# MattAgostini/ECE1782-Smith-Waterman-CUDA

Hardware: AMD Instinct MI355X
Metric: GCUPS (DP cell updates/s) query-vs-SwissProt, 1/2/4/8 MI355X; bit-exact scores (higher is better)
Workload: dtype fp16

## Files before the change

ece1782-smith-waterman-cuda_amd/csrc/sw_capi.cpp:

```cpp
#include <hip/hip_runtime.h>

#include <algorithm>
#include <cmath>
#include <atomic>
#include <cstdio>
#include <cstdlib>
#include <cstring>
#include <numeric>
#include <string>
#include <thread>
#include <unordered_map>
#include <vector>

#include "sw_amd.h"
#include "sw_kernels.h"
#include "sw_plan.h"

namespace {

thread_local std::string g_err;

constexpr int kF16Span = 2048;

uint32_t f16_pair(int v) {
// ... 1126 lines not shown
        HIPCHECK(hipHostGetDevicePointer(reinterpret_cast<void**>(&a.trace), db->h_trace, 0));
    }
    if (p.rescue) {
        a.rescue_count = c.listA;
        a.rescue_list = c.listA + 1;
        if (p.f16) a.rescue_max = c.maxA;
        const int zero = -kF16Span + 2 * ge;
        a.sat_limit = kF16Span - zero - 2 * std::max(c.sc.max_s, 1) - 26 * ge;
        for (int j = 0; j < 32; ++j) a.f16_step[j] = f16_pair(j * ge + zero);
        a.f16_gog = f16_pair(go - ge);
        a.f16_zero = f16_pair(zero);
        a.f16_diff[0] = f16_pair(4 * ge);
        a.f16_diff[1] = f16_pair(8 * ge);
        a.f16_diff[2] = f16_pair(16 * ge);
    }
    if (p.lpt) {
        a.blk_first = p.npair;
        a.blk_quad = p.nquad;
        a.blk_tri = p.ntri ? 1 : 0;
        a.blk_tail = static_cast<int32_t>(db->nblocks) - p.ntail;
    } else if (p.npair) {
        a.blk_base = p.nr;
        a.blk_first = std::max(p.npair, p.nr);
    } else {
        a.blk_first = p.ncoop;
    }
    return SW_OK;
}

void intra_args(Scan& c) {
// ... 40 lines not shown
    return c.db->nblocks ? inter_args(c) : SW_OK;
}

struct RescueStages {
    swk::InterArgs a16, a32;
    swk::IntraArgs i16, i32;
};
RescueStages rescue_stages(const Scan& c, const swk::IntraArgs& x, const BndRows& r, bool in_launch) {
    const swplan::ScanPlan& p = c.plan;
    auto items = [](int32_t* list) { return list ? list + 1 : nullptr; };
    int32_t* const l32 = p.f16 ? c.listB : c.listA;
    RescueStages s{c.a, c.a, x, c.ia};
    s.a16.bnd_h = s.a32.bnd_h = r.h;
    s.a16.bnd_f = s.a32.bnd_f = r.f;
    s.a16.qpad = p.qpad_list;
    s.a16.rescue_list = items(c.listB);
    s.a16.rescue_count = c.listB;
    s.a16.rescue_max = nullptr;
    s.a32.prof = c.P.dev + c.P.off8;
    s.a32.qpad = p.qpad_rescue;
    s.a32.rescue_list = nullptr;
    s.a32.rescue_count = nullptr;
    s.i16.bnd_h = s.i32.bnd_h = r.lh;
    s.i16.bnd_f = s.i32.bnd_f = r.lf;
    s.i16.rescue_list = items(c.list2);
    s.i16.rescue_count = c.list2;
    if (in_launch) {
        s.a16.trace = s.a32.trace = nullptr;
        s.a32.rescue_max = nullptr;
    } else {
// ... 1113 lines not shown
```

ece1782-smith-waterman-cuda_amd/csrc/sw_int32.h:

```cpp
#pragma once

#include "sw_kernels.h"

namespace swk {

__host__ __device__ constexpr int inter_stride(int R) {
    return ((R + 16 + 15) / 16) % 2 == 1 ? ((R + 16 + 15) / 16) * 16
                                         : ((R + 16 + 15) / 16 + 1) * 16;
}

__device__ __forceinline__ int sx8(uint32_t w, int b) {
    return static_cast<int>(static_cast<int8_t>(w >> (8 * b)));
}

__device__ __forceinline__ int usub(int m, uint32_t g) {
    return static_cast<int>(__builtin_elementwise_sub_sat(static_cast<uint32_t>(m), g));
}

template <int N>
__device__ __forceinline__ uint32_t pword(const int4 (&v)[N], int w) {
    const int4 q = v[w >> 2];
    switch (w & 3) {
        case 0: return static_cast<uint32_t>(q.x);
        case 1: return static_cast<uint32_t>(q.y);
// ... 237 lines not shown
template <int RI, bool AFFINE, bool WG = true>
__device__ __forceinline__ void intra_subject(const IntraArgs& a, int sid, uint8_t* lds) {
    auto sync = [] {
        if constexpr (WG) {
            __syncthreads();
        } else {
            __builtin_amdgcn_fence(__ATOMIC_RELEASE, "workgroup");
            __builtin_amdgcn_wave_barrier();
            __builtin_amdgcn_fence(__ATOMIC_ACQUIRE, "workgroup");
        }
    };
    constexpr int CH = kLanes * RI;
    constexpr int RIP = intra_rip(RI);
    constexpr int S = intra_stride(RI);
    constexpr int CHUNK_BYTES = kProfileRows * kLanes * RIP;
    const int lane = threadIdx.x & (kLanes - 1);
    const int L = a.subj_len[sid];
    const uint8_t* __restrict__ res = a.residues + a.subj_off[sid];
    int32_t* bnd_h = a.bnd_h + a.subj_off[sid];
    int32_t* bnd_f = AFFINE ? a.bnd_f + a.subj_off[sid] : nullptr;
    const uint32_t go = static_cast<uint32_t>(a.gap_open);
    const uint32_t ge = static_cast<uint32_t>(a.gap_extend);
    int best = 0;

    for (int c0 = 0, ch = 0; c0 < a.qpad; c0 += CH, ++ch) {
        const bool first = (c0 == 0);
        const bool last = (c0 + CH >= a.qpad);
        sync();
        const int8_t* src = a.prof + static_cast<size_t>(ch) * CHUNK_BYTES;
        for (int t = lane; t < CHUNK_BYTES / 16; t += kLanes) {
            const int c = t / (kLanes * RIP / 16);
// ... 95 lines not shown
```

ece1782-smith-waterman-cuda_amd/csrc/sw_inter_x2.hip:

```cpp
#include <algorithm>

#include "sw_int32.h"
#include "sw_intra_x2.h"
#include "sw_kernels.h"

namespace swk {

typedef short s2 __attribute__((ext_vector_type(2)));
typedef unsigned short u2 __attribute__((ext_vector_type(2)));

__device__ __forceinline__ s2 as_s2(uint32_t x) { return __builtin_bit_cast(s2, x); }
__device__ __forceinline__ uint32_t as_u32(s2 x) { return __builtin_bit_cast(uint32_t, x); }
__device__ __forceinline__ s2 max2(s2 a, s2 b) { return __builtin_elementwise_max(a, b); }
__device__ __forceinline__ s2 usub2(s2 a, u2 g) {
    return __builtin_bit_cast(s2, __builtin_elementwise_sub_sat(__builtin_bit_cast(u2, a), g));
}

__host__ __device__ constexpr int x2_row_dwords(int R) { return (R / 4) % 2 == 1 ? R : R + 4; }

constexpr int kImgCodes = kPadCode + 1;

template <int R>
struct __attribute__((aligned(16))) X2Lds {
    static constexpr int kImg = kImgCodes * x2_row_dwords(R);
// ... 86 lines not shown
        uint16_t* p = reinterpret_cast<uint16_t*>(bnd) + i;
        uint32_t w[SG / 2];
#pragma unroll
        for (int q = 0; q < SG / 2; ++q) w[q] = lo_lo(hb[2 * q], hb[2 * q + 1]);
        if constexpr (SG == 8) *reinterpret_cast<int4*>(p) = make_int4(w[0], w[1], w[2], w[3]);
        else *reinterpret_cast<int2*>(p) = make_int2(w[0], w[1]);
    }
}

__device__ __forceinline__ uint32_t to_f16_bits(uint32_t v16) {
    return static_cast<uint32_t>(__builtin_bit_cast(uint16_t, static_cast<_Float16>(static_cast<int16_t>(v16))));
}

template <int R, bool F16>
__device__ __forceinline__ void stage_x2s(X2Lds<R>& L, const int16_t* __restrict__ prof, int stride, int s0,
                                          int lane, int bias, int bias0, int img) {
    constexpr int RD = x2_row_dwords(R);
    constexpr int PER = kImgCodes * (R / 8);
    constexpr uint32_t one = F16 ? 0x3c00u : 1u;
    const int n = img < 0 ? 2 * PER : PER;
    for (int t = lane; t < n; t += kLanes) {
        const int im = img < 0 ? t / PER : img;
        const int u = img < 0 ? t % PER : t;
        const int c = u / (R / 8);
        const int k = u % (R / 8);
        const int4 v = *reinterpret_cast<const int4*>(prof + static_cast<size_t>(c) * stride + s0 + im * R + 8 * k);
        const uint32_t w[4] = {static_cast<uint32_t>(v.x), static_cast<uint32_t>(v.y), static_cast<uint32_t>(v.z),
                               static_cast<uint32_t>(v.w)};
        uint32_t o[8];
#pragma unroll
        for (int e = 0; e < 4; ++e) {
            const int s0v = static_cast<int16_t>(w[e] & 0xffffu), s1v = static_cast<int16_t>(w[e] >> 16);
            const int b0 = (F16 && k % 2 == 0 && e == 0) ? bias0 : 0;
            uint32_t a0 = static_cast<uint32_t>(s0v) & 0xffffu, a1 = static_cast<uint32_t>(s1v) & 0xffffu;
            if constexpr (F16) {
                a0 = to_f16_bits(static_cast<uint32_t>(s0v + bias + b0));
                a1 = to_f16_bits(static_cast<uint32_t>(s1v + bias));
            }
            o[2 * e] = im ? (a0 << 16) | one : a0 | (one << 16);
            o[2 * e + 1] = im ? (a1 << 16) | one : a1 | (one << 16);
        }
// ... 35 lines not shown
    static __device__ __forceinline__ V from(uint32_t x) { return as_s2(x); }
    static __device__ __forceinline__ uint32_t bits(V x) { return as_u32(x); }
};

template <>
struct PkCell<true> {
    using V = h2;
    static __device__ __forceinline__ V from(uint32_t x) { return __builtin_bit_cast(h2, x); }
    static __device__ __forceinline__ uint32_t bits(V x) { return __builtin_bit_cast(uint32_t, x); }
};

__device__ __forceinline__ h2 max3h(h2 a, h2 b, h2 c) {
    return __builtin_elementwise_maximum(__builtin_elementwise_maximum(a, b), c);
}

template <int R, int SG, bool AFFINE, bool F16, int CR = 16>
__device__ __forceinline__ bool x2s_block(const InterArgs& a, int blk, X2Lds<R>& L, int lane);

template <int R, int SG, bool AFFINE, bool F16, bool LIST, int CR = 16>
__global__ __launch_bounds__(256, 2) void sw_inter_x2s(InterArgs a) {
    static_assert(R % CR == 0 && SG % 4 == 0, "shape");
    __shared__ __attribute__((aligned(16))) X2Lds<R> lds[kWavesPerWG];
    const int wave = __builtin_amdgcn_readfirstlane(threadIdx.x >> 6);
    const int lane = threadIdx.x & 63;
    X2Lds<R>& L = lds[wave];
    if constexpr (LIST) {
        const int n = __builtin_amdgcn_readfirstlane(*a.blk_count);
        for (int i = blockIdx.x * kWavesPerWG + wave; i < n; i += gridDim.x * kWavesPerWG)
            x2s_block<R, SG, AFFINE, F16, CR>(a, list_take(a.blk_list, i), L, lane);
        return;
    }
    const int blk = a.blk_first + blockIdx.x * kWavesPerWG + wave;
    if (blk >= a.nblocks) return;
    x2s_block<R, SG, AFFINE, F16, CR>(a, blk, L, lane);
}

constexpr int kRowGroup = 16;
constexpr int kAcc = kRowGroup + 8 - 1;
template <bool F16>
struct Best {
    typename PkCell<F16>::V v;
    __device__ __forceinline__ void init(const InterArgs&) { v = PkCell<F16>::from(0u); }
    __device__ __forceinline__ typename PkCell<F16>::V value(const InterArgs&) const { return v; }
};
// ... 95 lines not shown
constexpr bool pair_flags() { return AFFINE; }
struct PairSync {
    int* prog;
    int me;
    int base;
    int pred;
    int pred_base;
    int succ;
    int S;
};
__device__ __forceinline__ void pair_wait(const int* prog, int wave, int need) {
    while (__hip_atomic_load(prog + wave, __ATOMIC_ACQUIRE, __HIP_MEMORY_SCOPE_WORKGROUP) < need)
        __builtin_amdgcn_s_sleep(1);
}

template <int R, int SG, bool AFFINE, bool F16, bool PAIR, int CR = 16, bool CHAIN = false>
__device__ __forceinline__ void x2s_pass(const InterArgs& a, X2Lds<R>& L, uint32_t ncols, uint64_t base, int lane,
                                         int s0, Best<F16>& best, const int4* ring_in, int4* ring_out,
                                         int* tick, const PairSync* ps = nullptr) {
    static_assert(!(CHAIN && PAIR), "chained passes: single-wave blocks only");
    constexpr int CQ = CR / 4;
    constexpr int NCH = R / CR;
    constexpr int STEPS = SG * NCH;
    using P = PkCell<F16>;
    using V = typename P::V;
    const int16_t* prof16 = reinterpret_cast<const int16_t*>(a.prof);
    const u2 go2 = {static_cast<unsigned short>(a.gap_open), static_cast<unsigned short>(a.gap_open)};
    const u2 ge2 = {static_cast<unsigned short>(a.gap_extend), static_cast<unsigned short>(a.gap_extend)};
    uint32_t* bnd = reinterpret_cast<uint32_t*>(a.bnd_h);
    static_assert(!F16 || (R % kRowGroup == 0 && SG <= 8), "fp16 row groups");
    h2 gog_h = {}, reb_h = {}, grp_h = {};
    if constexpr (F16) {
        gog_h = __builtin_bit_cast(h2, a.f16_gog);
        static_assert(SG == 4 || SG == 8, "rebase constants");
        reb_h = __builtin_bit_cast(h2, a.f16_diff[SG == 4 ? 0 : 1]);
        grp_h = __builtin_bit_cast(h2, a.f16_diff[2]);
    }
    const bool first = (s0 == 0);
    const bool last = (s0 + 2 * R >= a.qpad);
    const uint32_t npass = CHAIN ? static_cast<uint32_t>((a.qpad + 2 * R - 1) / (2 * R)) : 1u;
    const uint32_t total = npass * ncols;
    const int sbias = F16 ? (AFFINE ? 2 : 1) * a.gap_extend : 0;
    const int gbias0 = F16 ? -kRowGroup * a.gap_extend : 0;
    const uint32_t dtop0 = F16 ? a.f16_step[SG - 2 + kRowGroup] : 0u;
    stage_x2s<R, F16>(L, prof16, a.prof_stride, s0, lane, sbias, gbias0, -1);
    __builtin_amdgcn_fence(__ATOMIC_RELEASE, "workgroup");
    __builtin_amdgcn_wave_barrier();
    __builtin_amdgcn_fence(__ATOMIC_ACQUIRE, "workgroup");

    V H[R];
    V E[AFFINE ? R : 1];
#pragma unroll
    for (int r = 0; r < R; ++r) H[r] = P::from(F16 ? a.f16_step[r % kRowGroup + SG - 1] : 0u);
#pragma unroll
    for (int r = 0; r < (AFFINE ? R : 1); ++r) E[r] = P::from(F16 ? a.f16_zero : 0u);
    uint32_t dtop = dtop0;
    uint32_t dl_h[SG], dl_f[SG];
    uint32_t bin[SG], bin_n[SG];
    uint32_t bz[SG];
    uint32_t rc[SG / 4], rp[SG / 4], rn[SG / 4];
// ... 11 lines not shown
    for (int q = 0; q < SG / 4; ++q) rp[q] = 0x19191919u;
    load_codes<SG>(rc, a.residues + base, true);
    constexpr bool kPairFlags = pair_flags<AFFINE>();
    auto wait_in = [&](uint32_t x) {
        if constexpr (PAIR && kPairFlags)
            pair_wait(ps->prog, ps->pred, ps->pred_base + min(static_cast<int>(x) + 2, ps->S));
    };
    if (!first) {
        wait_in(0);
        if (PAIR && ring_in) ring_load<SG>(bin, ring_in, 0, lane);
        else load_bnd<SG, AFFINE>(bin, bnd, base);
    }
    int4 PL[2][CQ], PH[2][CQ];
    constexpr uint32_t RB = x2_row_dwords(R) * 4;
    const uint32_t blo = lds_addr(L.lo), bhi = lds_addr(L.hi);
    uint32_t aa = code_row<RB>(rc, 0, blo), ab = code_row<RB>(rp, 0, bhi);
    read_x2a<CQ>(PL[0], PH[0], aa, ab, 0, 0);

    uint32_t lo_p = 0, lo_c = 0;
    bool t2 = false;
    for (uint32_t col0 = 0; col0 <= total; col0 += SG) {
        const bool has_next = col0 + SG <= total;
        const bool next_lo = col0 + SG < total;
        const uint32_t ncol = col0 + SG;
        const bool wrap = CHAIN && lo_c + SG == ncols;
        const uint32_t nreal = CHAIN ? (wrap ? 0u : lo_c + SG) : ncol;
        const bool next_first = CHAIN ? (lo_p == 0 && !wrap) : first;
        const uint64_t noff = (nreal >> 4) * kGroupBytes + (nreal & 15);
        const bool t1 = CHAIN && lo_c == 0 && lo_p > 0 && lo_p < npass;
        const bool next_t1 = CHAIN && wrap && next_lo;
        const bool next_t2 = t1;
// ... 28 lines not shown
        if (next_t1) {
            __builtin_amdgcn_fence(__ATOMIC_RELEASE, "workgroup");
            __builtin_amdgcn_fence(__ATOMIC_ACQUIRE, "workgroup");
        }
        if (has_next) {
            load_codes<SG>(rn, a.residues + base + noff, next_lo);
            if (!next_first && next_lo) {
                wait_in(ncol / SG);
                if (PAIR && ring_in) ring_load<SG>(bin_n, ring_in, (ncol / SG) % kRingSlots, lane);
                else load_bnd<SG, AFFINE>(bin_n, bnd, base + noff);
            }
        }
        if constexpr (F16) {
#pragma unroll
            for (int r = 0; r < R; ++r) {
                H[r] = H[r] - reb_h;
                if constexpr (AFFINE) E[r] = E[r] - reb_h;
            }
            dtop = P::bits(P::from(dtop) - reb_h);
        }
        auto cell = [&](const int r, const int jj, V& up, V& diag, V& f, const V slo, const V shi) {
            if constexpr (F16 && !AFFINE) {
                const int rg = r % kRowGroup;
                if (rg == 0 && r > 0) up = up - grp_h;
                const h2 t = max3h(H[r], up, __builtin_elementwise_fma(slo, shi, diag));
                const h2 h = __builtin_elementwise_maximum(t, __builtin_bit_cast(h2, a.f16_step[rg + jj]));
                h2& acc = best.acc[rg + jj];
                if (jj & 1) {
                    if (rg + 1 < kRowGroup) acc = max3h(acc, h, H[r + 1]);
                    else acc = __builtin_elementwise_maximum(acc, h);
                } else if (rg == 0) {
                    acc = __builtin_elementwise_maximum(acc, h);
// ... 27 lines not shown
            E[r] = __builtin_elementwise_maximum(E[r], m);
            f = max3h(f, m, __builtin_bit_cast(h2, a.f16_step[rg + jj + 1]));
            h2& acc = best.acc[rg + jj];
            if (jj & 1) {
                if (rg + 1 < kRowGroup) acc = max3h(acc, h, H[r + 1]);
                else acc = __builtin_elementwise_maximum(acc, h);
            } else if (rg == 0) {
                acc = __builtin_elementwise_maximum(acc, h);
            }
            diag = H[r];
            H[r] = h;
            up = h;
          }
        };
        auto col_done = [&](const V up, const V f, const int jj) {
            dl_h[jj] = P::bits(up);
            if constexpr (AFFINE) dl_f[jj] = P::bits(f);
        };
        auto col_start = [&](V& up, V& diag, V& f, const int jj) {
            const uint32_t u = (AFFINE || jj % 2 == 0) ? lo_lo(bin[jj], dl_h[jj]) : hi_lo(bin[jj], dl_h[jj]);
            up = P::from(u);
            if constexpr (F16 && !AFFINE) up = up - grp_h;
            diag = P::from(dtop);
            dtop = u;
            if constexpr (AFFINE) f = P::from(hi_lo(bin[jj], dl_f[jj]));
            if constexpr (F16) f = f - grp_h;
        };
        V up = P::from(0u), diag = P::from(0u), f = P::from(0u);
#pragma unroll
        for (int t = 0; t < STEPS; ++t) {
            const int jj = t / NCH;
            const int k = t % NCH;
// ... 1 lines not shown
            if (t + 1 < STEPS) {
                const int jn = (t + 1) / NCH, kn = (t + 1) % NCH;
                if (kn == 0) {
                    aa = code_row<RB>(rc, jn, blo);
                    ab = code_row<RB>(rp, jn, bhi);
                }
                read_x2a<CQ>(PL[(t + 1) & 1], PH[(t + 1) & 1], aa, ab, kn, dep);
            } else if (has_next && !next_t1 && !next_t2) {
                aa = code_row<RB>(rn, 0, blo);
                ab = code_row<RB>(rc, 0, bhi);
                read_x2a<CQ>(PL[(t + 1) & 1], PH[(t + 1) & 1], aa, ab, 0, dep);
            }
            if (k == 0) col_start(up, diag, f, jj);
            const int4(&pl)[CQ] = PL[t & 1];
            const int4(&ph)[CQ] = PH[t & 1];
            if constexpr (F16 && AFFINE) {
                V dd[CR];
#pragma unroll
                for (int i = 0; i < CR; ++i)
                    dd[i] = __builtin_elementwise_fma(P::from(word(pl, i)), P::from(word(ph, i)),
                                                      i == 0 ? diag : H[CR * k + i - 1]);
#pragma unroll
                for (int i = 0; i < CR; ++i) asm volatile("" : "+v"(dd[i]));
#pragma unroll
                for (int i = 0; i < CR; ++i) cell_d(CR * k + i, jj, up, diag, f, dd[i]);
            } else {
#pragma unroll
                for (int i = 0; i < CR; ++i)
                    cell(CR * k + i, jj, up, diag, f, P::from(word(pl, i)), P::from(word(ph, i)));
            }
            if (k == NCH - 1) col_done(up, f, jj);
            if constexpr (!F16) asm volatile("" : "+v"(best.v));
            else best.pin();
            __builtin_amdgcn_sched_barrier(0);
        }
        const bool high_last = CHAIN ? (lo_c == 0 ? lo_p : lo_p + 1) >= npass : last;
        if (!high_last && col0 >= SG) {
            uint32_t hb[SG];
#pragma unroll
            for (int q = 0; q < SG; ++q) hb[q] = AFFINE ? hi_hi(dl_h[q], dl_f[q]) : hi_hi(dl_h[q], dl_h[q]);
            const uint32_t pc = CHAIN ? (lo_c == 0 ? ncols - SG : lo_c - SG) : col0 - SG;
            if (PAIR && ring_out) {
                if constexpr (kPairFlags) {
                    const int x = static_cast<int>(pc / SG);
                    pair_wait(ps->prog, ps->succ, x >= kRingSlots ? ps->base + x - kRingSlots + 1 : ps->base - 2);
                }
                ring_store<SG>(ring_out, (pc / SG) % kRingSlots, lane, hb);
            } else {
                const uint64_t poff = (pc >> 4) * kGroupBytes + (pc & 15);
                store_bnd<SG, AFFINE>(bnd, base + poff, hb);
            }
// ... 15 lines not shown
            __syncthreads();
            ++*tick;
        }
        if constexpr (CHAIN) {
            t2 = t1;
            lo_c = nreal;
            lo_p += wrap ? 1u : 0u;
        }
    }
}

__device__ __forceinline__ uint32_t block_cols(const InterArgs& a, int blk) {
    return a.blk_cols ? a.blk_cols[blk] : a.blk_groups[blk] * kGroupCols;
}

template <int R, int SG, bool AFFINE, bool F16, int CR>
__device__ __forceinline__ bool x2s_block(const InterArgs& a, int blk, X2Lds<R>& L, int lane) {
    const uint32_t ncols = block_cols(a, blk);
    const uint64_t base = a.blk_off[blk] + static_cast<uint64_t>(lane) * kGroupCols;
    Best<F16> best;
    best.init(a);
    const uint64_t t0 = trace_now();
    if (ncols >= 32 && a.qpad > 2 * R) {
        x2s_pass<R, SG, AFFINE, F16, false, CR, true>(a, L, ncols, base, lane, 0, best, nullptr, nullptr, nullptr);
    } else {
        for (int s0 = 0; s0 < a.qpad && ncols > 0; s0 += 2 * R)
            x2s_pass<R, SG, AFFINE, F16, false, CR>(a, L, ncols, base, lane, s0, best, nullptr, nullptr, nullptr);
    }
    const bool flagged = x2s_finish<F16>(a, blk, lane, best.value(a));
    trace_block(a, blk, t0, lane, 0);
    return flagged;
}

constexpr int kPairLag = 3;
constexpr int kPairCR = 8;
constexpr int kSingleCR = 8;
constexpr int kGroupWavesPerEU = 2;

__device__ __forceinline__ int group_ticks(uint32_t ncols, int passes, int SG, int G) {
    if (ncols == 0 || passes <= 0) return 0;
    const int S = static_cast<int>(ncols) / SG + 1;
    const int per = max(S, G * kPairLag);
// ... 20 lines not shown
    using P = PkCell<F16>;
    using V = typename P::V;
    const int tid = tid_x();
    const int wave = __builtin_amdgcn_readfirstlane(tid >> 6);
    const int lane = tid & 63;
    const int npair = MERGED ? a.blk_first : a.nblocks;
    const int qend = GMAX == 4 ? quad_end : a.blk_base;
    const int qwg = qend - a.blk_base;
    const int pwg = qwg + (npair - qend + 1) / 2;
    const int tail = MERGED && a.blk_tail > npair && a.blk_tail < a.nblocks ? a.blk_tail : a.nblocks;
    const bool tri_on = MERGED && GMAX == 4 && AFFINE && a.blk_tri != 0;
    const int nspare = tri_on ? max(0, min(qwg, tail - npair)) : 0;
    const int s0 = npair + nspare;
    const int twg = pwg + (tail - s0 + kWavesPerWG - 1) / kWavesPerWG;
    const bool tailp = MERGED && wgi >= twg;
    if (MERGED && wgi >= pwg && !tailp) {
        const int blk = s0 + (wgi - pwg) * kWavesPerWG + wave;
        return blk < tail && x2s_block<R, SG, AFFINE, F16, kSingleCR>(a, blk, lds[wave], lane);
    }
    const bool quad = !tailp && wgi < qwg;
    const bool tri = tri_on && quad;
    const bool spare = tri && wave == kWavesPerWG - 1;
    const int G = tri ? 3 : quad ? 4 : 2, NG = tri ? 1 : kWavesPerWG / G;
    const int first = quad ? a.blk_base + wgi : tailp ? tail + (wgi - twg) * 2 : qend + (wgi - qwg) * 2;
    const int gend = tailp ? a.nblocks : npair;
    const int gi = spare ? 0 : wave / G, w = spare ? 0 : wave % G;
    const int passes = (a.qpad + 2 * R - 1) / (2 * R);
    int tmax = 0;
    for (int q = 0; q < NG; ++q) {
        const int b = first + q;
        if (b < gend) tmax = max(tmax, group_ticks(block_cols(a, b), passes, SG, G));
    }
    const int blk = first + gi;
    Best<F16> best;
    best.init(a);
    int tick = 0;
    const uint64_t t0 = trace_now();
    constexpr bool kPairFlags = pair_flags<AFFINE>();
    if constexpr (kPairFlags) {
        if (tid < kWavesPerWG) sm.prog[tid] = 0;
        __syncthreads();
    }
    bool flagged = false;
    if (spare) {
        const int sb = npair + wgi;
        if (sb < s0) flagged = x2s_block<R, SG, AFFINE, F16, kSingleCR>(a, sb, lds[wave], lane);
    } else if (blk < gend) {
        const uint32_t ncols = block_cols(a, blk);
        const uint64_t base = a.blk_off[blk] + static_cast<uint64_t>(lane) * kGroupCols;
        const int per = max(static_cast<int>(ncols) / SG + 1, G * kPairLag);
        const int4* rin = w > 0 ? ring[gi * (G - 1) + w - 1] : nullptr;
        int4* rout = w < G - 1 ? ring[gi * (G - 1) + w] : nullptr;
        PairSync ps{sm.prog, wave, 0, -1, 0, w < G - 1 ? wave + 1 : -1, static_cast<int>(ncols) / SG + 1};
        for (int p = w; p < passes && ncols > 0; p += G) {
            if constexpr (kPairFlags) {
                const int k = p / G;
                ps.base = k * ps.S;
                ps.pred = p == 0 ? -1 : w > 0 ? wave - 1 : wave + G - 1;
                ps.pred_base = (w > 0 ? k : k - 1) * ps.S;
            } else {
                const int start = (p / G) * per + kPairLag * w;
                while (tick < start) {
                    __syncthreads();
                    ++tick;
                }
            }
            x2s_pass<R, SG, AFFINE, F16, true, kPairCR>(a, lds[wave], ncols, base, lane, p * 2 * R, best, rin, rout,
                                                        &tick, &ps);
        }
    }
    (void)tmax;
    if constexpr (!kPairFlags) {
        while (tick < tmax) {
            __syncthreads();
            ++tick;
        }
    }
    if (!spare && blk < gend && w > 0) part[wave][lane] = P::bits(best.value(a));
    __syncthreads();
    if (!spare && blk < gend && w == 0) {
        V b = best.value(a);
        for (int u = 1; u < G; ++u) {
            const V o = P::from(part[wave + u][lane]);
// ... 19 lines not shown
    static constexpr int R32 = AFFINE ? 32 : 64;
};
template <bool AFFINE, int RI>
constexpr size_t drain_smem() {
    using D = DrainShape<AFFINE>;
    const size_t x16 = kWavesPerWG * sizeof(X2Lds<D::R16>);
    const size_t i32 = static_cast<size_t>(kProfileRows) * intra_stride(RI);
    const size_t a32 = static_cast<size_t>(kWavesPerWG) * kProfileRows * inter_stride(D::R32);
    const size_t i16 = sizeof(typename ix2::IntraImg<RI, false>::Elem) * ix2::img_elems<RI, false>();
    return std::max(std::max(x16, i32), std::max(a32, i16));
}

template <bool AFFINE, int RI>
__device__ __forceinline__ void lpt_drain(const DrainArgs* __restrict__ d, char* smem, int* task) {
    using D = DrainShape<AFFINE>;
    const int wave = __builtin_amdgcn_readfirstlane(threadIdx.x >> 6);
    const int lane = threadIdx.x & 63;
    for (;;) {
        __syncthreads();
        if (threadIdx.x == 0) {
            constexpr int kOrder[4] = {2, 0, 3, 1};
            constexpr int kWant[4] = {2 * kWavesPerWG, kWavesPerWG, 1, kWavesPerWG};
            int kind = 0, n = 0, start = 0;
            for (int k = 0; k < 4 && !n; ++k) {
                const int l = kOrder[k];
                if ((n = list_claim(d->lists[l], d->heads[l], kWant[k], &start))) kind = l + 1;
            }
            int m = 0;
            for (int i = 0; i < n; ++i) {
                const int v = list_wait_take(d->lists[kind - 1] + 1, start + i, d->fault, d->spin);
                if (v >= 0) task[2 + m++] = v;
            }
            task[0] = m ? kind : (n ? -1 : 0);
            task[1] = m;
        }
        __syncthreads();
        const int kind = task[0], n = task[1];
        if (kind == 0) return;
        if (kind < 0) continue;
        __builtin_amdgcn_fence(__ATOMIC_ACQUIRE, "agent");
        if (kind == 3) {
            IntraArgs y = d->i16;
            y.subj_list = task + 2;
            y.list_count = task + 1;
            ix2::intra_x2_wg<RI, false, true, !AFFINE, false, false, false, true>(y, 0,
                                                               reinterpret_cast<typename ix2::IntraImg<RI, false>::Elem*>(smem));
        } else if (kind == 1) {
            if (wave < n)
                x2s_block<D::R16, D::SG16, AFFINE, false, 16>(d->a16, task[2 + wave],
                                                              reinterpret_cast<X2Lds<D::R16>*>(smem)[wave], lane);
        } else if (kind == 4) {
            if (wave == 0) intra_subject<RI, AFFINE, false>(d->i32, task[2], reinterpret_cast<uint8_t*>(smem));
        } else {
            if (wave < n)
                inter_block<D::R32, 8, AFFINE, false>(
                    d->a32, task[2 + wave],
                    reinterpret_cast<uint8_t*>(smem) + wave * (kProfileRows * inter_stride(D::R32)), lane);
        }
    }
}

struct LptParams {
    InterArgs a;
    IntraArgs ia;
// ... 24 lines not shown
        const InterArgs& a = p.a;
        const IntraArgs& ia = p.ia;
        const int niwg = ((ia.nsubj + 1) / 2 + kWavesPerWG - 1) / kWavesPerWG;
        const int item = p.order[k];
        const uint64_t t0 = trace_now();
        bool flagged;
        if (item >= 0)
            flagged = x2p_wg<R, SG, AFFINE, true, true, 4>(a, item, a.blk_quad,
                                                           *reinterpret_cast<X2pSmem<R, SG, 4>*>(smem));
        else if (-1 - item < niwg)
            flagged = ix2::intra_x2_wg<RI, true, false, !AFFINE, true, false, AFFINE, true>(
                ia, -1 - item, reinterpret_cast<Elem*>(smem));
        else
            flagged = ix2::intra_x2_wg<2, true, false, !AFFINE, true, true, AFFINE, true>(
                ia, -1 - item - niwg, reinterpret_cast<PElem*>(smem));
        const bool any = __syncthreads_or(flagged);
        if (threadIdx.x == 0) trace_block(a, a.nblocks + k, t0, 0, item >= 0 ? 2 : 3);
        if (p.drain && any) lpt_drain<AFFINE, RI>(p.drain, smem, task);
        if constexpr (!LOOP) break;
        if (threadIdx.x == 0) claimed = p.grid + __hip_atomic_fetch_add(p.next, 1, __ATOMIC_RELAXED, __HIP_MEMORY_SCOPE_AGENT);
        __syncthreads();
        k = claimed;
        __syncthreads();
        if (k >= p.n) break;
    }
}

template <int R, int RI, bool AFFINE>
static int lpt_slots(int cus) {
    static const int per = [] {
        int p = 0;
// ... 94 lines not shown
```

ece1782-smith-waterman-cuda_amd/csrc/sw_kernels.h:

```cpp
#pragma once

#include <hip/hip_runtime.h>
#include <stdint.h>

#include <string>

#include "sw_amd.h"

namespace swk {

int set_error(int code, const std::string& msg);

constexpr int kLanes = 64;
constexpr int kGroupCols = 16;
constexpr int kGroupBytes = kLanes * kGroupCols;
constexpr int kProfileRows = 32;
constexpr int kPadCode = 25;
constexpr uint8_t kStored[26] = {11, 1, 5, 2, 22, 6, 14, 12, 23, 9, 10, 0, 24, 7, 4, 15, 3, 21, 8, 13, 16, 17, 18, 19, 20, 25};
constexpr uint8_t kCodeOf[26] = {11, 1, 3, 16, 14, 2, 5, 13, 18, 9, 10, 0, 7, 19, 6, 15, 20, 21, 22, 23, 24, 17, 4, 8, 12, 25};
constexpr int kWavesPerWG = 4;
constexpr int kIntraSteps = 40;

template <int SG>
struct Residues {
// ... 31 lines not shown
    int32_t* rescue_count;
    const int32_t* blk_list;
    const int32_t* blk_count;
    int32_t blk_first;
    int32_t sat_limit;
    uint32_t f16_step[32];
    uint32_t f16_gog;
    uint32_t f16_zero;
    uint32_t f16_diff[3];
    int32_t blk_base;
    int32_t blk_quad;
    int32_t blk_tri;
    int32_t blk_tail;
    int32_t* rescue_max;
    uint64_t* trace;
};

struct IntraArgs {
    const uint8_t* residues;
    const uint64_t* subj_off;
    const int32_t* subj_len;
    const int32_t* subj_id;
    int32_t nsubj;
    const int8_t* prof;
    int32_t qpad;
    int32_t gap_open;
    int32_t gap_extend;
    int32_t* bnd_h;
    int32_t* bnd_f;
    int32_t* scores;
// ... 168 lines not shown
```

ece1782-smith-waterman-cuda_amd/csrc/sw_plan.cpp:

```cpp
#include "sw_plan.h"

#include <algorithm>
#include <cmath>
#include <cstdio>
#include <utility>
#include <vector>

namespace swplan {

namespace {
int32_t round_up(int64_t v, int64_t m) { return static_cast<int32_t>((v + m - 1) / m * m); }
}


constexpr int64_t kSmallDbSubjects = 64 * 1000;

constexpr double kFillSubjects = 570000.0;

int32_t default_long_threshold(const PlanDb& db) {
    if (db.n == 0) return 1536;
    const double mean = static_cast<double>(db.residues) / static_cast<double>(db.n);
    if (db.n < kSmallDbSubjects && mean >= 256) return 64;
    const double fill = db.n < kSmallDbSubjects ? 1.0 : std::min(1.0, static_cast<double>(db.n) / kFillSubjects);
    const double t = 5.7 * mean * std::pow(fill, 0.4);
// ... 220 lines not shown
    for (int ri : {4, 6, 8, 10, 12, 16, swk::kIntraX2MaxRI}) {
        if (ri == swk::kIntraX2MaxRI && wide < 2) continue;
        const int chunk = swk::kLanes * ri;
        const int nch = (qlen + chunk - 1) / chunk;
        const double cost = static_cast<double>(nch) * (longest + swk::kLanes - 1) * (ri * 28.8 + 80.0);
        if (cost < best_cost) {
            best_cost = cost;
            best_ri = ri;
        }
    }
    return best_ri;
}

bool lpt_supported(int ri) { return ri == 4 || ri == 6 || ri == 8; }

PlanScoring plan_scoring(const int8_t* m, int go, int ge) {
    PlanScoring s;
    s.go = go;
    s.ge = ge;
    for (int k = 0; k < 625; ++k) {
        s.max_s = std::max<int>(s.max_s, m[k]);
        if (m[k] + go > 127) s.biased_fits = false;
    }
    return s;
}

ScanPlan scan_plan(const PlanDb& db, int32_t qlen, const PlanScoring& s, bool intra_i16_first, int32_t i16_span) {
    const sw_opts& O = *db.opts;
    const int max_s = s.max_s, go = s.go, ge = s.ge;
    ScanPlan p;
// ... 18 lines not shown
        db.nblocks == 0 && 2 * max_s + (swk::intra_bias_rows(swk::kIntraX2MaxRI) + 1) * ge + go < 1024;
    const int ri2_model =
        p.intra_x2 ? intra_x2_rows_for(qlen, db.long_max, ri2_wide ? (affine ? 2 : 1) : 0, O.intra_x2_rows) : 0;
    const int ri2_lpt = (affine && ri2_model > 8 && db.nblocks && O.intra_x2_rows < 0) ? 8 : ri2_model;

    p.npair = (db.nblocks && swk::inter_has_pair(p.shape) && round_up(qlen, R) > R) ? pair_blocks(db) : 0;
    p.ncoop = (!p.npair && db.nblocks) ? coop_blocks(db, swk::inter_coop_divisor(p.shape)) : 0;
    p.qpad_coop = p.ncoop ? round_up(qlen, swk::kCoopRows) : 0;
    p.nr = (p.f16 && p.rescue && p.npair && !p.ncoop) ? i16_span : 0;

    const bool lpt_want = O.lpt >= 0 ? O.lpt == 1 : true;
    p.lpt = lpt_want && db.nlong && db.nblocks && p.intra_x2 && !p.intra_i16_first && p.f16 && p.rescue &&
            p.npair && !p.ncoop && i16_span == 0 && lpt_supported(ri2_lpt);
    p.lpt_rows = (p.lpt && !affine && O.lpt_rows != 64 && round_up(qlen, 96) > 96) ? 96 : 64;
    p.qpad_inter = round_up(qlen, p.lpt_rows == 96 ? 96 : R);
    if (p.lpt) {
        const int passes = p.qpad_inter / p.lpt_rows;
        p.ntri = affine ? lpt_tri_blocks(db, p.npair, passes) : 0;
        p.nquad = p.ntri ? p.ntri : lpt_quad_blocks(db, p.npair);
        p.ntail = lpt_tail_blocks(db, p.npair, passes);
    }

    p.ri = db.nlong ? intra_rows_for(qlen, db.long_max) : 0;
    p.qpad_intra = p.ri ? round_up(qlen, static_cast<int64_t>(swk::kLanes) * p.ri) : 0;
    p.ri2 = p.lpt ? ri2_lpt : ri2_model;
    p.qpad_intra2 = p.ri2 ? round_up(qlen, static_cast<int64_t>(swk::kLanes) * p.ri2) : 0;
    p.multi_inter = p.qpad_inter > R || p.qpad_rescue > rescue_rows(affine) || p.qpad_coop > swk::kCoopRows ||
                    p.qpad_list > list_rows;
    p.multi_intra = (p.ri && p.qpad_intra > swk::kLanes * p.ri) || (p.ri2 && p.qpad_intra2 > swk::kLanes * p.ri2);

// ... 26 lines not shown
```

ece1782-smith-waterman-cuda_amd/csrc/sw_plan.h:

```cpp
#pragma once

#include <cstdint>
#include <string>
#include <vector>

#include "sw_amd.h"
#include "sw_kernels.h"

namespace swplan {

struct PlanDb {
    int64_t n = 0;
    int64_t residues = 0;
    int64_t nblocks = 0;
    int64_t nlong = 0;
    int32_t long_threshold = 0;
    int32_t long_max = 0;
    const uint32_t* blk_groups = nullptr;
    const int32_t* llen = nullptr;
    const sw_opts* opts = nullptr;
    int cus = 0;
};

int32_t default_long_threshold(const PlanDb& db);
// ... 1 lines not shown
int pair_group(const PlanDb& db);
int32_t pair_blocks(const PlanDb& db);
int32_t lpt_quad_blocks(const PlanDb& db, int32_t npair);
int32_t lpt_tri_blocks(const PlanDb& db, int32_t npair, int passes);
int32_t lpt_tail_blocks(const PlanDb& db, int32_t npair, int passes);
double intra_step_us(int ri);
double single_ticks(int64_t ncols, int passes);
double group_ticks_host(int64_t ncols, int passes, int G);

swk::InterShape inter_shape(bool affine, int x2_ok, const sw_opts& o);
std::string inter_kernel_name(const swk::InterShape& v, bool affine);
int rescue_rows(bool affine);
int intra_rows_for(int qlen, int longest);
int intra_x2_rows_for(int qlen, int longest, int wide, int forced);
bool lpt_supported(int ri);

struct PlanScoring {
    int max_s = 0;
    int go = 0, ge = 0;
    bool biased_fits = true;
};
PlanScoring plan_scoring(const int8_t* matrix625, int go, int ge);

struct ScanPlan {
    bool affine = false;
    int x2_ok = 0;
    swk::InterShape shape{};
    bool rescue = false;
    bool f16 = false;
    bool intra_x2 = false;
    bool intra_i16_first = false;
    int ri = 0;
    int ri2 = 0;
    int32_t qpad_inter = 0, qpad_intra = 0, qpad_intra2 = 0, qpad_rescue = 0, qpad_list = 0, qpad_coop = 0;
    int32_t npair = 0;
    int32_t ncoop = 0;
    int32_t nr = 0;
    bool lpt = false;
    bool drain = false;
    int lpt_rows = 64;
    int32_t ntri = 0, nquad = 0, ntail = 0;
    bool multi_inter = false, multi_intra = false;
    std::string kernel, intra_kernel;

    void set_drain(bool got_rows);
};

ScanPlan scan_plan(const PlanDb& db, int32_t qlen, const PlanScoring& s, bool intra_i16_first, int32_t i16_span);

struct LptPlan {
    std::vector<int32_t> order;
    std::vector<float> cost;
    int32_t npipe = 0;
    int32_t pipe_tail = 0;
};
// ... 5 lines not shown
```

Before: 11080.

## Run a shortened final strip pass when query padding leaves spare rows

Adds a plan-computed re_last row count so the last query strip of the inter x2 kernels can run with R-4 rows per half instead of R when the query remainder fits. The short pass skips DP cells in padded rows, restages the profile with an offset stride, and rebiases boundary values for f16. Chained passes are also split so that the short strip runs separately. It additionally replaces __syncthreads_or with a ballot-plus-LDS reduction in the LPT loop. This adds template instantiations, code size and correctness risk around the boundary bias.

```diff
diff --git a/ece1782-smith-waterman-cuda_amd/csrc/sw_capi.cpp b/ece1782-smith-waterman-cuda_amd/csrc/sw_capi.cpp
--- a/ece1782-smith-waterman-cuda_amd/csrc/sw_capi.cpp
+++ b/ece1782-smith-waterman-cuda_amd/csrc/sw_capi.cpp
@@ -1164,6 +1164,7 @@
         a.f16_diff[1] = f16_pair(8 * ge);
         a.f16_diff[2] = f16_pair(16 * ge);
     }
+    a.re_last = p.re_last;
     if (p.lpt) {
         a.blk_first = p.npair;
         a.blk_quad = p.nquad;
@@ -1234,6 +1235,8 @@
     s.a16.bnd_h = s.a32.bnd_h = r.h;
     s.a16.bnd_f = s.a32.bnd_f = r.f;
     s.a16.qpad = p.qpad_list;
+    s.a16.re_last = p.affine ? 32 : 48;
+    s.a32.re_last = swplan::rescue_rows(p.affine);
     s.a16.rescue_list = items(c.listB);
     s.a16.rescue_count = c.listB;
     s.a16.rescue_max = nullptr;
diff --git a/ece1782-smith-waterman-cuda_amd/csrc/sw_int32.h b/ece1782-smith-waterman-cuda_amd/csrc/sw_int32.h
--- a/ece1782-smith-waterman-cuda_amd/csrc/sw_int32.h
+++ b/ece1782-smith-waterman-cuda_amd/csrc/sw_int32.h
@@ -275,7 +275,7 @@
     constexpr int RIP = intra_rip(RI);
     constexpr int S = intra_stride(RI);
     constexpr int CHUNK_BYTES = kProfileRows * kLanes * RIP;
-    const int lane = threadIdx.x & (kLanes - 1);
+    const int lane = tid_x() & (kLanes - 1);
     const int L = a.subj_len[sid];
     const uint8_t* __restrict__ res = a.residues + a.subj_off[sid];
     int32_t* bnd_h = a.bnd_h + a.subj_off[sid];
diff --git a/ece1782-smith-waterman-cuda_amd/csrc/sw_inter_x2.hip b/ece1782-smith-waterman-cuda_amd/csrc/sw_inter_x2.hip
--- a/ece1782-smith-waterman-cuda_amd/csrc/sw_inter_x2.hip
+++ b/ece1782-smith-waterman-cuda_amd/csrc/sw_inter_x2.hip
@@ -124,7 +124,7 @@
 
 template <int R, bool F16>
 __device__ __forceinline__ void stage_x2s(X2Lds<R>& L, const int16_t* __restrict__ prof, int stride, int s0,
-                                          int lane, int bias, int bias0, int img) {
+                                          int lane, int bias, int bias0, int img, int hi0 = R) {
     constexpr int RD = x2_row_dwords(R);
     constexpr int PER = kImgCodes * (R / 8);
     constexpr uint32_t one = F16 ? 0x3c00u : 1u;
@@ -134,7 +134,14 @@
         const int u = img < 0 ? t % PER : t;
         const int c = u / (R / 8);
         const int k = u % (R / 8);
-        const int4 v = *reinterpret_cast<const int4*>(prof + static_cast<size_t>(c) * stride + s0 + im * R + 8 * k);
+        const int16_t* src = prof + static_cast<size_t>(c) * stride + s0 + im * hi0 + 8 * k;
+        int4 v;
+        if (im && (hi0 & 7)) {
+            const int2 v0 = *reinterpret_cast<const int2*>(src), v1 = *reinterpret_cast<const int2*>(src + 4);
+            v = make_int4(v0.x, v0.y, v1.x, v1.y);
+        } else {
+            v = *reinterpret_cast<const int4*>(src);
+        }
         const uint32_t w[4] = {static_cast<uint32_t>(v.x), static_cast<uint32_t>(v.y), static_cast<uint32_t>(v.z),
                                static_cast<uint32_t>(v.w)};
         uint32_t o[8];
@@ -200,7 +207,7 @@
     return __builtin_elementwise_maximum(__builtin_elementwise_maximum(a, b), c);
 }
 
-template <int R, int SG, bool AFFINE, bool F16, int CR = 16>
+template <int R, int SG, bool AFFINE, bool F16, int CR = 16, bool SHORT = true>
 __device__ __forceinline__ bool x2s_block(const InterArgs& a, int blk, X2Lds<R>& L, int lane);
 
 template <int R, int SG, bool AFFINE, bool F16, bool LIST, int CR = 16>
@@ -213,7 +220,7 @@
     if constexpr (LIST) {
         const int n = __builtin_amdgcn_readfirstlane(*a.blk_count);
         for (int i = blockIdx.x * kWavesPerWG + wave; i < n; i += gridDim.x * kWavesPerWG)
-            x2s_block<R, SG, AFFINE, F16, CR>(a, list_take(a.blk_list, i), L, lane);
+            x2s_block<R, SG, AFFINE, F16, CR, false>(a, list_take(a.blk_list, i), L, lane);
         return;
     }
     const int blk = a.blk_first + blockIdx.x * kWavesPerWG + wave;
@@ -339,10 +346,10 @@
         __builtin_amdgcn_s_sleep(1);
 }
 
-template <int R, int SG, bool AFFINE, bool F16, bool PAIR, int CR = 16, bool CHAIN = false>
+template <int R, int SG, bool AFFINE, bool F16, bool PAIR, int CR = 16, bool CHAIN = false, int RL = R>
 __device__ __forceinline__ void x2s_pass(const InterArgs& a, X2Lds<R>& L, uint32_t ncols, uint64_t base, int lane,
                                          int s0, Best<F16>& best, const int4* ring_in, int4* ring_out,
-                                         int* tick, const PairSync* ps = nullptr) {
+                                         int* tick, const PairSync* ps = nullptr, int chain_passes = 1) {
     static_assert(!(CHAIN && PAIR), "chained passes: single-wave blocks only");
     constexpr int CQ = CR / 4;
     constexpr int NCH = R / CR;
@@ -363,12 +370,19 @@
     }
     const bool first = (s0 == 0);
     const bool last = (s0 + 2 * R >= a.qpad);
-    const uint32_t npass = CHAIN ? static_cast<uint32_t>((a.qpad + 2 * R - 1) / (2 * R)) : 1u;
+    const uint32_t npass = CHAIN ? static_cast<uint32_t>(chain_passes) : 1u;
+    const bool chain_last = CHAIN && static_cast<int>(npass) * 2 * R >= a.qpad;
     const uint32_t total = npass * ncols;
     const int sbias = F16 ? (AFFINE ? 2 : 1) * a.gap_extend : 0;
     const int gbias0 = F16 ? -kRowGroup * a.gap_extend : 0;
     const uint32_t dtop0 = F16 ? a.f16_step[SG - 2 + kRowGroup] : 0u;
-    stage_x2s<R, F16>(L, prof16, a.prof_stride, s0, lane, sbias, gbias0, -1);
+    constexpr bool kSh = RL < R;
+    if constexpr (kSh) asm volatile("" : "+v"(lane));
+    static_assert(!kSh || (RL == R - 4 && !CHAIN), "rows per strip: R, or R - 4 outside a chain");
+    static_assert((R - 4 - 1) % kRowGroup == 11, "the short strip's bottom row: 4 ge under the last row's bias");
+    h2 dsh_h = {};
+    if constexpr (F16) dsh_h = __builtin_bit_cast(h2, a.f16_diff[0]);
+    stage_x2s<R, F16>(L, prof16, a.prof_stride, s0, lane, sbias, gbias0, -1, RL);
     __builtin_amdgcn_fence(__ATOMIC_RELEASE, "workgroup");
     __builtin_amdgcn_wave_barrier();
     __builtin_amdgcn_fence(__ATOMIC_ACQUIRE, "workgroup");
@@ -410,7 +424,7 @@
     int4 PL[2][CQ], PH[2][CQ];
     constexpr uint32_t RB = x2_row_dwords(R) * 4;
     const uint32_t blo = lds_addr(L.lo), bhi = lds_addr(L.hi);
-    uint32_t aa = code_row<RB>(rc, 0, blo), ab = code_row<RB>(rp, 0, bhi);
+    uint32_t aa = code_row<RB>(rc, 0, blo), ab = bhi + kPadCode * RB;
     read_x2a<CQ>(PL[0], PH[0], aa, ab, 0, 0);
 
     uint32_t lo_p = 0, lo_c = 0;
@@ -469,8 +483,9 @@
         if constexpr (F16) {
 #pragma unroll
             for (int r = 0; r < R; ++r) {
-                H[r] = H[r] - reb_h;
-                if constexpr (AFFINE) E[r] = E[r] - reb_h;
+                if (r <= RL) H[r] = H[r] - reb_h;
+                if constexpr (AFFINE)
+                    if (r < RL) E[r] = E[r] - reb_h;
             }
             dtop = P::bits(P::from(dtop) - reb_h);
         }
@@ -528,8 +543,13 @@
           }
         };
         auto col_done = [&](const V up, const V f, const int jj) {
-            dl_h[jj] = P::bits(up);
-            if constexpr (AFFINE) dl_f[jj] = P::bits(f);
+            if constexpr (kSh && F16) {
+                dl_h[jj] = P::bits(up + dsh_h);
+                if constexpr (AFFINE) dl_f[jj] = P::bits(f + dsh_h);
+            } else {
+                dl_h[jj] = P::bits(up);
+                if constexpr (AFFINE) dl_f[jj] = P::bits(f);
+            }
         };
         auto col_start = [&](V& up, V& diag, V& f, const int jj) {
             const uint32_t u = (AFFINE || jj % 2 == 0) ? lo_lo(bin[jj], dl_h[jj]) : hi_lo(bin[jj], dl_h[jj]);
@@ -561,27 +581,31 @@
             if (k == 0) col_start(up, diag, f, jj);
             const int4(&pl)[CQ] = PL[t & 1];
             const int4(&ph)[CQ] = PH[t & 1];
+            const int n = RL - CR * k < CR ? (RL - CR * k > 0 ? RL - CR * k : 0) : CR;
             if constexpr (F16 && AFFINE) {
                 V dd[CR];
 #pragma unroll
                 for (int i = 0; i < CR; ++i)
-                    dd[i] = __builtin_elementwise_fma(P::from(word(pl, i)), P::from(word(ph, i)),
-                                                      i == 0 ? diag : H[CR * k + i - 1]);
-#pragma unroll
-                for (int i = 0; i < CR; ++i) asm volatile("" : "+v"(dd[i]));
-#pragma unroll
-                for (int i = 0; i < CR; ++i) cell_d(CR * k + i, jj, up, diag, f, dd[i]);
+                    if (i < n)
+                        dd[i] = __builtin_elementwise_fma(P::from(word(pl, i)), P::from(word(ph, i)),
+                                                          i == 0 ? diag : H[CR * k + i - 1]);
+#pragma unroll
+                for (int i = 0; i < CR; ++i)
+                    if (i < n) asm volatile("" : "+v"(dd[i]));
+#pragma unroll
+                for (int i = 0; i < CR; ++i)
+                    if (i < n) cell_d(CR * k + i, jj, up, diag, f, dd[i]);
             } else {
 #pragma unroll
                 for (int i = 0; i < CR; ++i)
-                    cell(CR * k + i, jj, up, diag, f, P::from(word(pl, i)), P::from(word(ph, i)));
+                    if (i < n) cell(CR * k + i, jj, up, diag, f, P::from(word(pl, i)), P::from(word(ph, i)));
             }
             if (k == NCH - 1) col_done(up, f, jj);
             if constexpr (!F16) asm volatile("" : "+v"(best.v));
             else best.pin();
             __builtin_amdgcn_sched_barrier(0);
         }
-        const bool high_last = CHAIN ? (lo_c == 0 ? lo_p : lo_p + 1) >= npass : last;
+        const bool high_last = CHAIN ? chain_last && (lo_c == 0 ? lo_p : lo_p + 1) >= npass : last;
         if (!high_last && col0 >= SG) {
             uint32_t hb[SG];
 #pragma unroll
@@ -627,18 +651,28 @@
     return a.blk_cols ? a.blk_cols[blk] : a.blk_groups[blk] * kGroupCols;
 }
 
-template <int R, int SG, bool AFFINE, bool F16, int CR>
+template <int R, int SG, bool AFFINE, bool F16, int CR, bool SHORT>
 __device__ __forceinline__ bool x2s_block(const InterArgs& a, int blk, X2Lds<R>& L, int lane) {
     const uint32_t ncols = block_cols(a, blk);
     const uint64_t base = a.blk_off[blk] + static_cast<uint64_t>(lane) * kGroupCols;
     Best<F16> best;
     best.init(a);
     const uint64_t t0 = trace_now();
-    if (ncols >= 32 && a.qpad > 2 * R) {
-        x2s_pass<R, SG, AFFINE, F16, false, CR, true>(a, L, ncols, base, lane, 0, best, nullptr, nullptr, nullptr);
-    } else {
-        for (int s0 = 0; s0 < a.qpad && ncols > 0; s0 += 2 * R)
-            x2s_pass<R, SG, AFFINE, F16, false, CR>(a, L, ncols, base, lane, s0, best, nullptr, nullptr, nullptr);
+    const bool sh = SHORT && a.re_last == R - 4 && (ncols < 32 || ncols >= 64);
+    const int full_end = a.qpad - (sh ? 2 * R : 0);
+    const int chained = ncols >= 32 ? full_end / (2 * R) : 0;
+    int s0 = 0;
+    if (chained > 1) {
+        x2s_pass<R, SG, AFFINE, F16, false, CR, true>(a, L, ncols, base, lane, 0, best, nullptr, nullptr, nullptr,
+                                                      nullptr, chained);
+        s0 = chained * 2 * R;
+    }
+    for (; s0 < full_end && ncols > 0; s0 += 2 * R)
+        x2s_pass<R, SG, AFFINE, F16, false, CR>(a, L, ncols, base, lane, s0, best, nullptr, nullptr, nullptr);
+    if constexpr (SHORT) {
+        if (sh && ncols > 0)
+            x2s_pass<R, SG, AFFINE, F16, false, CR, false, R - 4>(a, L, ncols, base, lane, full_end, best, nullptr,
+                                                                  nullptr, nullptr);
     }
     const bool flagged = x2s_finish<F16>(a, blk, lane, best.value(a));
     trace_block(a, blk, t0, lane, 0);
@@ -689,10 +723,7 @@
     const int s0 = npair + nspare;
     const int twg = pwg + (tail - s0 + kWavesPerWG - 1) / kWavesPerWG;
     const bool tailp = MERGED && wgi >= twg;
-    if (MERGED && wgi >= pwg && !tailp) {
-        const int blk = s0 + (wgi - pwg) * kWavesPerWG + wave;
-        return blk < tail && x2s_block<R, SG, AFFINE, F16, kSingleCR>(a, blk, lds[wave], lane);
-    }
+    const bool singles = MERGED && wgi >= pwg && !tailp;
     const bool quad = !tailp && wgi < qwg;
     const bool tri = tri_on && quad;
     const bool spare = tri && wave == kWavesPerWG - 1;
@@ -717,17 +748,18 @@
         __syncthreads();
     }
     bool flagged = false;
-    if (spare) {
-        const int sb = npair + wgi;
-        if (sb < s0) flagged = x2s_block<R, SG, AFFINE, F16, kSingleCR>(a, sb, lds[wave], lane);
-    } else if (blk < gend) {
+    const int sb = singles ? s0 + (wgi - pwg) * kWavesPerWG + wave : npair + wgi;
+    if ((singles && sb < tail) || (spare && sb < s0))
+        flagged = x2s_block<R, SG, AFFINE, F16, kSingleCR>(a, sb, lds[wave], lane);
+    if (singles) return flagged;
+    if (!spare && blk < gend) {
         const uint32_t ncols = block_cols(a, blk);
         const uint64_t base = a.blk_off[blk] + static_cast<uint64_t>(lane) * kGroupCols;
         const int per = max(static_cast<int>(ncols) / SG + 1, G * kPairLag);
         const int4* rin = w > 0 ? ring[gi * (G - 1) + w - 1] : nullptr;
         int4* rout = w < G - 1 ? ring[gi * (G - 1) + w] : nullptr;
         PairSync ps{sm.prog, wave, 0, -1, 0, w < G - 1 ? wave + 1 : -1, static_cast<int>(ncols) / SG + 1};
-        for (int p = w; p < passes && ncols > 0; p += G) {
+        auto enter = [&](const int p) {
             if constexpr (kPairFlags) {
                 const int k = p / G;
                 ps.base = k * ps.S;
@@ -740,8 +772,18 @@
                     ++tick;
                 }
             }
+        };
+        const int pfull = passes - (a.re_last == R - 4 ? 1 : 0);
+        int p = w;
+        for (; p < pfull && ncols > 0; p += G) {
+            enter(p);
             x2s_pass<R, SG, AFFINE, F16, true, kPairCR>(a, lds[wave], ncols, base, lane, p * 2 * R, best, rin, rout,
                                                         &tick, &ps);
+        }
+        if (p == pfull && pfull < passes && ncols > 0) {
+            enter(p);
+            x2s_pass<R, SG, AFFINE, F16, true, kPairCR, false, R - 4>(a, lds[wave], ncols, base, lane, p * 2 * R, best,
+                                                                      rin, rout, &tick, &ps);
         }
     }
     (void)tmax;
@@ -791,11 +833,12 @@
 template <bool AFFINE, int RI>
 __device__ __forceinline__ void lpt_drain(const DrainArgs* __restrict__ d, char* smem, int* task) {
     using D = DrainShape<AFFINE>;
-    const int wave = __builtin_amdgcn_readfirstlane(threadIdx.x >> 6);
-    const int lane = threadIdx.x & 63;
     for (;;) {
+        const int tid = tid_x();
+        const int wave = __builtin_amdgcn_readfirstlane(tid >> 6);
+        const int lane = tid & 63;
         __syncthreads();
-        if (threadIdx.x == 0) {
+        if (tid == 0) {
             constexpr int kOrder[4] = {2, 0, 3, 1};
             constexpr int kWant[4] = {2 * kWavesPerWG, kWavesPerWG, 1, kWavesPerWG};
             int kind = 0, n = 0, start = 0;
@@ -824,7 +867,7 @@
                                                                reinterpret_cast<typename ix2::IntraImg<RI, false>::Elem*>(smem));
         } else if (kind == 1) {
             if (wave < n)
-                x2s_block<D::R16, D::SG16, AFFINE, false, 16>(d->a16, task[2 + wave],
+                x2s_block<D::R16, D::SG16, AFFINE, false, 16, false>(d->a16, task[2 + wave],
                                                               reinterpret_cast<X2Lds<D::R16>*>(smem)[wave], lane);
         } else if (kind == 4) {
             if (wave == 0) intra_subject<RI, AFFINE, false>(d->i32, task[2], reinterpret_cast<uint8_t*>(smem));
@@ -879,7 +922,11 @@
         else
             flagged = ix2::intra_x2_wg<2, true, false, !AFFINE, true, true, AFFINE, true>(
                 ia, -1 - item - niwg, reinterpret_cast<PElem*>(smem));
-        const bool any = __syncthreads_or(flagged);
+        const int tw = tid_x();
+        const bool wany = __builtin_amdgcn_ballot_w64(flagged) != 0;
+        if ((tw & 63) == 0) task[2 + (tw >> 6)] = wany;
+        __syncthreads();
+        const bool any = (task[2] | task[3] | task[4] | task[5]) != 0;
         if (threadIdx.x == 0) trace_block(a, a.nblocks + k, t0, 0, item >= 0 ? 2 : 3);
         if (p.drain && any) lpt_drain<AFFINE, RI>(p.drain, smem, task);
         if constexpr (!LOOP) break;
diff --git a/ece1782-smith-waterman-cuda_amd/csrc/sw_kernels.h b/ece1782-smith-waterman-cuda_amd/csrc/sw_kernels.h
--- a/ece1782-smith-waterman-cuda_amd/csrc/sw_kernels.h
+++ b/ece1782-smith-waterman-cuda_amd/csrc/sw_kernels.h
@@ -69,6 +69,7 @@
     int32_t blk_tail;
     int32_t* rescue_max;
     uint64_t* trace;
+    int32_t re_last;
 };
 
 struct IntraArgs {
diff --git a/ece1782-smith-waterman-cuda_amd/csrc/sw_plan.cpp b/ece1782-smith-waterman-cuda_amd/csrc/sw_plan.cpp
--- a/ece1782-smith-waterman-cuda_amd/csrc/sw_plan.cpp
+++ b/ece1782-smith-waterman-cuda_amd/csrc/sw_plan.cpp
@@ -258,6 +258,11 @@
 
 bool lpt_supported(int ri) { return ri == 4 || ri == 6 || ri == 8; }
 
+int32_t short_rows(int32_t qlen, int pass_rows) {
+    const int32_t left = qlen - (round_up(qlen, pass_rows) / pass_rows - 1) * pass_rows;
+    return (left + 1) / 2 <= pass_rows / 2 - 4 ? pass_rows / 2 - 4 : pass_rows / 2;
+}
+
 PlanScoring plan_scoring(const int8_t* m, int go, int ge) {
     PlanScoring s;
     s.go = go;
@@ -306,6 +311,7 @@
             p.npair && !p.ncoop && i16_span == 0 && lpt_supported(ri2_lpt);
     p.lpt_rows = (p.lpt && !affine && O.lpt_rows != 64 && round_up(qlen, 96) > 96) ? 96 : 64;
     p.qpad_inter = round_up(qlen, p.lpt_rows == 96 ? 96 : R);
+    p.re_last = p.shape.x2s ? short_rows(qlen, p.lpt_rows == 96 ? 96 : R) : 0;
     if (p.lpt) {
         const int passes = p.qpad_inter / p.lpt_rows;
         p.ntri = affine ? lpt_tri_blocks(db, p.npair, passes) : 0;
diff --git a/ece1782-smith-waterman-cuda_amd/csrc/sw_plan.h b/ece1782-smith-waterman-cuda_amd/csrc/sw_plan.h
--- a/ece1782-smith-waterman-cuda_amd/csrc/sw_plan.h
+++ b/ece1782-smith-waterman-cuda_amd/csrc/sw_plan.h
@@ -39,6 +39,7 @@
 int intra_rows_for(int qlen, int longest);
 int intra_x2_rows_for(int qlen, int longest, int wide, int forced);
 bool lpt_supported(int ri);
+int32_t short_rows(int32_t qlen, int pass_rows);
 
 struct PlanScoring {
     int max_s = 0;
@@ -64,6 +65,7 @@
     bool lpt = false;
     bool drain = false;
     int lpt_rows = 64;
+    int32_t re_last = 0;
     int32_t ntri = 0, nquad = 0, ntail = 0;
     bool multi_inter = false, multi_intra = false;
     std::string kernel, intra_kernel;
```

Result: faster. 11320, median of 6 (+2.2%).
